# sxontheway/milliEye

Hardware: AMD Instinct MI355X
Metric: frames/sec YOLOv3-416+fusion @batch32, 1/2/4/8 MI355X; mAP@0.5 vs ref (higher is better)
Workload: dtype f32; 1 GPU; yolov3.cfg 416x416 fp32 inference, batch=32 per GPU, full milliEye: Darknet.forward -> NMS -> Network.forward mode 0 (R-CNN head + radar fusion, 2 radar boxes/frame) -> output rows, synthetic frames U[0,1), deterministic trained-like weights; stage=full, batch_per_gpu=32, global_batch=32, img_size=416, parallelism=frames sharded over 1 GPU(s), one process per GPU, no data-path collective, rccl_ranks=0, full=False, output_rows_last_step=6449, rois_last_step=6449

## Files before the change

millieye_amd/csrc/conv.hip:

```cpp
#include <stdlib.h>

#include "common.h"
#include "dma.h"

#include "conv32_common.h"

namespace me32 {
int launch_p8_tile(const ConvP& p, int tile, hipStream_t stream);
bool ws1x1_f32_eligible(const ConvP& p);
int launch_ws1x1_f32(const ConvP& p, hipStream_t stream);
bool ws3x3_f32_eligible(const ConvP& p);
int launch_ws3x3_f32(const ConvP& p, hipStream_t stream);
bool stem_mfma_eligible(const ConvP& p);
int launch_stem_mfma(const ConvP& p, hipStream_t stream);
}

namespace {

template <int BM, int BN, int BK, int WR, int WC, int ABL = 0, int PRIO = 0>
__global__ __launch_bounds__(256) void conv_igemm_f32(ConvP p) {
  static_assert(WR * WC == 4, "4 waves per workgroup");
  constexpr int TM = BM / WR, TN = BN / WC;
  constexpr int MT = TM / 32, NT = TN / 32;
  static_assert(MT >= 1 && NT >= 1, "wave tile must hold at least one 32x32 MFMA tile");
  constexpr int LP = BK + 4;
  constexpr int CH = BK / 4;
  constexpr int A_IT = (BM * CH + 255) / 256;
  constexpr int B_IT = (BN * CH + 255) / 256;

  extern __shared__ __attribute__((aligned(16))) float smem[];
  float* As = smem;
  float* Bs = smem + 2 * BM * LP;

  const int tid = threadIdx.x;
  const int lane = tid & 63;
  const int wave = tid >> 6;
  const int wr = wave / WC, wc = wave % WC;
  const int r32 = lane & 31, hh = lane >> 5;

  int tile_m, tile_n;
  {
    const int nwg = p.tiles_m * p.tiles_n;
    const int bid = blockIdx.x;
    const int q = nwg >> 3, r = nwg & 7;
    const int xcd = bid & 7, idx = bid >> 3;
    const int wg = (xcd < r ? xcd * (q + 1) : r * (q + 1) + (xcd - r) * q) + idx;
    tile_n = wg % p.tiles_n;
// ... 1305 lines not shown

extern "C" {

int64_t me_conv2d_flops(const me_conv_desc* d) {
  if (!d) return 0;
  return 2ll * d->n * d->ho * d->wo * (int64_t)d->cout * d->ksize * d->ksize * d->cin;
}

int64_t me_conv2d_workspace_bytes(const me_conv_desc* d) {
  ConvP p;
  if (!d || fill_params(d, p) != 0 || d->cin <= 4) return 0;
  if ((d->tile >= 41 && d->tile <= 45) || d->tile == 47) {
    static const int shape[7][2] = {{128, 128}, {128, 64}, {64, 64}, {128, 32}, {256, 128}, {0, 0}, {64, 64}};
    const int bm = shape[d->tile - 41][0], bn = shape[d->tile - 41][1];
    const long long tiles = (long long)((p.M + bm - 1) / bm) * ((p.cout + bn - 1) / bn);
    const int split = d->split_k > 0 ? d->split_k : 4;
    return (int64_t)(tiles % 256) * split * bm * bn * (int64_t)sizeof(float);
  }
  const ConvPlan plan = plan_conv(p, d->tile, d->split_k > 0 ? d->split_k : kMaxSplit);
  const int split = d->split_k > 0 ? d->split_k : plan.splitk;
  return split > 1 ? (int64_t)split * p.M * p.cout * (int64_t)sizeof(float) : 0;
}

int me_conv2d_f32(const me_conv_desc* d, void* stream_) {
  hipStream_t stream = reinterpret_cast<hipStream_t>(stream_);
  ConvP p;
  int rc = fill_params(d, p);
  if (rc) return rc;
  ME_REQUIRE(d->x && d->wgt && d->scale && d->shift && d->y, ME_E_NULLPTR, "me_conv2d_f32: null tensor pointer");
  ME_REQUIRE(d->upsample == 1 || d->upsample == 2, ME_E_BADARG, "me_conv2d_f32: upsample must be 1 or 2");
  ME_REQUIRE(d->act >= 0 && d->act <= 2, ME_E_BADARG, "me_conv2d_f32: unknown activation %d", d->act);
  ME_REQUIRE(d->y_pitch >= d->cout, ME_E_BADARG, "me_conv2d_f32: y_pitch < cout");

  if (d->cin <= 4) {
    ME_REQUIRE(d->ksize == 3, ME_E_BADARG, "me_conv2d_f32: cin <= 4 needs ksize 3 (direct stem kernel)");
    ME_REQUIRE(d->cout <= SC_MAXCOUT, ME_E_TOOBIG, "me_conv2d_f32: small-cin kernel supports cout <= %d", SC_MAXCOUT);
    ME_REQUIRE(d->res == nullptr && d->upsample == 1, ME_E_BADARG,
               "me_conv2d_f32: small-cin kernel has no residual/upsample epilogue");
    ME_REQUIRE(d->x_nchw || d->x_pitch >= d->cin, ME_E_BADARG, "me_conv2d_f32: x_pitch < cin");
    ME_REQUIRE(me::aligned16(d->y), ME_E_ALIGN, "me_conv2d_f32: y not 16-byte aligned");
    if (d->tile == 0 && me32::stem_mfma_eligible(p)) return me32::launch_stem_mfma(p, stream);
    if (d->cin == 3 && (d->y_pitch & 3) == 0 && d->tile != 91) {
      const unsigned mb = (unsigned)((p.M + 255) / 256);
      if (d->cout % 32 == 0) {
        hipLaunchKernelGGL(conv_stem3_f32<32>, dim3(mb, d->cout / 32), dim3(256), 0, stream, p);
        return me::check_launch("conv_stem3_f32");
      }
      if (d->cout % 16 == 0) {
        hipLaunchKernelGGL(conv_stem3_f32<16>, dim3(mb, d->cout / 16), dim3(256), 0, stream, p);
        return me::check_launch("conv_stem3_f32");
      }
    }
    const long long threads = (long long)p.M * (((p.cout + 7) & ~7) >> 3);
    const unsigned blocks = (unsigned)((threads + 255) / 256);
    if (d->cin == 3)
      hipLaunchKernelGGL(conv_smallcin_f32<3>, dim3(blocks), dim3(256), 0, stream, p);
    else
      hipLaunchKernelGGL(conv_smallcin_f32<4>, dim3(blocks), dim3(256), 0, stream, p);
    return me::check_launch("conv_smallcin_f32");
  }

  ME_REQUIRE(!d->x_nchw, ME_E_BADARG, "me_conv2d_f32: NCHW input only supported for cin <= 4");
  ME_REQUIRE(d->cin % 4 == 0, ME_E_BADARG, "me_conv2d_f32: cin %% 4 != 0 (cin=%d)", d->cin);
  ME_REQUIRE(d->x_pitch >= d->cin && d->x_pitch % 4 == 0, ME_E_ALIGN, "me_conv2d_f32: x_pitch must be >= cin, %% 4");
  ME_REQUIRE(me::aligned16(d->x) && me::aligned16(d->wgt), ME_E_ALIGN, "me_conv2d_f32: x / wgt not 16-byte aligned");
  ME_REQUIRE(!d->res || d->res_pitch >= d->cout, ME_E_BADARG, "me_conv2d_f32: res_pitch < cout");
// ... 90 lines not shown
```

millieye_amd/engine.py:

```python
import ctypes as C
import os

import torch

from . import hip

__all__ = ["DarknetEngine", "ConvWeights", "pick_tap_module", "invalidate_weights", "bump_versions"]

_ALIGN = 256

_EPOCH = [0]


def invalidate_weights():
    _EPOCH[0] += 1


def bump_versions(*tensors):
    torch.autograd.graph.increment_version(tensors)

_DTYPES = ("f32", "bf16", "f16")
_TORCH_HALF = {"bf16": torch.bfloat16, "f16": torch.float16}


def _resolve(idx, current):
    idx = int(idx)
    return current + idx if idx < 0 else idx


def pick_tap_module(module_defs):
    if len(module_defs) > 8 and module_defs[8]["type"] == "convolutional":
        return 8
    yolos = [i for i, d in enumerate(module_defs) if d["type"] == "yolo"]
    if len(yolos) < 2:
        return None
    tap = None
    for i in range(yolos[0] + 1, yolos[1]):
        d = module_defs[i]
        if d["type"] == "convolutional" and int(d["filters"]) == 256:
            tap = i
    return tap


class ConvWeights:

    def __init__(self, conv, bn=None, dtype="f32", cin_pad=0, cout_pad=0):
        self.conv, self.bn = conv, bn
        self.dtype, self.cin_pad, self.cout_pad = dtype, cin_pad, cout_pad
        self.wgt = self.scale = self.shift = None
        self.wgt_tiled = None
        self.want_rot = False
        self.rot = self.rot_tiled = None
        self.want_parity, self.parity, self.parity_stamp = False, None, None
        self._stamp = None

    def _sources(self):
        cp = self.conv._parameters
        ts = [cp["weight"]]
        if cp.get("bias") is not None:
            ts.append(cp["bias"])
        if self.bn is not None:
            bp, bb = self.bn._parameters, self.bn._buffers
            ts += [bp["weight"], bp["bias"], bb["running_mean"], bb["running_var"]]
        return ts

    def stamp(self):
        return tuple((t.data_ptr(), t._version) for t in self._sources()) + (_EPOCH[0],)

    def _prepare_packed_f32(self, device):
        conv, bn = self.conv, self.bn
        w = conv.weight
        cout, cin, k, k2 = w.shape
        if k != k2:
            return None
        srcs = [w] + [t for t in ((conv.bias,) if conv.bias is not None else ())]
        if bn is not None:
            srcs += [bn.weight, bn.bias, bn.running_mean, bn.running_var]
        if not all(t.device == device and t.dtype == torch.float32 and t.is_contiguous() for t in srcs):
            return None
        f32 = dict(device=device, dtype=torch.float32)
        realloc = self.wgt is None or self.wgt.device != device or tuple(self.wgt.shape) != (cout, k, k, cin) \
            or self.wgt.dtype != torch.float32
        if realloc:
            self.wgt = torch.empty((cout, k, k, cin), **f32)
            self.scale, self.shift = torch.empty(cout, **f32), torch.empty(cout, **f32)
            self.wgt_tiled = torch.empty((k * k, cin // 16, cout, 16), **f32) if cin % 16 == 0 else None
# ... 3 lines not shown
            self.rot_tiled = torch.empty((k * k, cout // 16, cin, 16), **f32) if cout % 16 == 0 else None
        if realloc:
            self.parity = None
        if self.want_parity and k == 3 and self.parity is None:
            self.parity = torch.empty((4 * cin, 2, 2, cout), **f32)
        return "realloc" if realloc else True

    def _pack_desc(self, d):
        conv, bn = self.conv, self.bn
        ptr = lambda t: t.data_ptr() if t is not None else None
        cout, cin, k, _ = conv.weight.shape
        d.w, d.bias = conv.weight.data_ptr(), ptr(conv.bias)
        d.gamma, d.beta = ptr(bn.weight if bn is not None else None), ptr(bn.bias if bn is not None else None)
        d.mean, d.var = ptr(bn.running_mean if bn is not None else None), ptr(bn.running_var if bn is not None else None)
        d.ohwi, d.tiled = self.wgt.data_ptr(), ptr(self.wgt_tiled)
        d.rot, d.rot_tiled = ptr(self.rot if self.want_rot else None), ptr(self.rot_tiled if self.want_rot else None)
        d.scale, d.shift = self.scale.data_ptr(), self.shift.data_ptr()
        d.parity = ptr(self.parity if self.want_parity else None)
        d.cout, d.cin, d.ksize, d.eps = cout, cin, k, float(bn.eps) if bn is not None else 0.0
        return d

    def _refresh_packed_f32(self, device):
        done = self._prepare_packed_f32(device)
        if done is None:
            return None
        self.parity_stamp = None
        d = self._pack_desc(hip.PackDesc())
        hip.check(hip.lib().me_pack_conv_f32(d.w, d.cout, d.cin, d.ksize, d.bias, d.gamma, d.beta, d.mean, d.var, d.eps, d.ohwi,
                                             d.tiled, d.rot, d.rot_tiled, d.scale, d.shift, hip.stream_ptr()),
                  "me_pack_conv_f32")
        return done

    def refresh(self, device):
        stamp = self.stamp() + (self.want_rot,)
        if stamp == self._stamp and self.wgt is not None and self.wgt.device == device:
            return False
        dev = torch.device(device)
        if self.dtype == "f32" and not self.cin_pad and not self.cout_pad and dev.type == "cuda":
            if dev.index is None:
                dev = torch.device("cuda", torch.cuda.current_device())
            done = self._refresh_packed_f32(dev)
            if done is not None:
                self._stamp = stamp
                return done
        with torch.no_grad():
            w = self.conv.weight.detach().to(device=device, dtype=torch.float32)
            packed = w.permute(0, 2, 3, 1).contiguous()
            cout = w.shape[0]
            if self.bn is not None:
                g = self.bn.weight.detach().to(device, torch.float64)
                b = self.bn.bias.detach().to(device, torch.float64)
                mean = self.bn.running_mean.detach().to(device, torch.float64)
                var = self.bn.running_var.detach().to(device, torch.float64)
                scale = g / torch.sqrt(var + self.bn.eps)
                shift = b - mean * scale
                if self.conv.bias is not None:
                    shift = shift + self.conv.bias.detach().to(device, torch.float64) * scale
            else:
                scale = torch.ones(cout, dtype=torch.float64, device=device)
                if self.conv.bias is not None:
                    shift = self.conv.bias.detach().to(device, torch.float64)
                else:
                    shift = torch.zeros(cout, dtype=torch.float64, device=device)
            scale, shift = scale.to(torch.float32), shift.to(torch.float32)
            cin = packed.shape[3]
            if self.cin_pad > cin:
# ... 401 lines not shown
        plan.arena = torch.empty(max(total, _ALIGN), dtype=torch.uint8, device=device)
        if plan.arena.data_ptr() % _ALIGN:
            raise RuntimeError("the caching allocator returned an arena that is not 256-byte aligned")
        plan.arena_bytes = total
        plan.dtype = self.dtype
        plan.rows = sum(yolo_rows)
        plan.num_classes = None
        base = plan.arena.data_ptr()

        def view(tt):
            root, coff = tt.root()
            return base + root.offset + tt.esize * coff, root.c

        def typed_view(tt, nchw):
            root, coff = tt.root()
            flat = plan.arena.view(_TORCH_HALF[self.dtype] if tt.esize == 2 else torch.float32)
            pitch, off = root.c, root.offset // tt.esize + coff
            if nchw:
                return torch.as_strided(flat, (n, tt.c, tt.h, tt.w), (tt.h * tt.w * pitch, 1, tt.w * pitch, pitch), off)
            return torch.as_strided(flat, (n, tt.h, tt.w, tt.c), (tt.h * tt.w * pitch, tt.w * pitch, pitch, 1), off)

        lib = hip.lib()
        launches = []
        plan.input_descs = []
        plan.yolo_raw = []
        plan.yolo_descs = []
        plan.conv_descs = []
        flops = 0
        for op in ops:
            kind = op["kind"]
            if kind == "conv":
                x, y = op["x"], op["y"]
                cw = self._conv_weights(op["module"], x.c if x.padded else 0, y.c if y.padded else 0)
                if cw.refresh(device) == "realloc" and self._plans:
                    self._plans.clear()
                dsc = hip.Conv16Desc() if bf16 else hip.ConvDesc()
                if x.external:
                    dsc.x, dsc.x_pitch, dsc.x_nchw = None, x.c, 1
                    plan.input_descs.append(dsc)
                else:
                    dsc.x, dsc.x_pitch = view(x)
                    dsc.x_nchw = 0
                dsc.wgt, dsc.scale, dsc.shift = cw.wgt.data_ptr(), cw.scale.data_ptr(), cw.shift.data_ptr()
                if op["res"] is not None:
                    dsc.res, dsc.res_pitch = view(op["res"])
                else:
                    dsc.res, dsc.res_pitch = None, 0
                dsc.y, dsc.y_pitch = view(y)
                dsc.n, dsc.h, dsc.w, dsc.cin = n, x.h, x.w, x.c
                dsc.cout, dsc.ksize, dsc.stride, dsc.pad = cw.wgt.shape[0], op["k"], op["s"], op["pad"]
                dsc.ho, dsc.wo, dsc.act, dsc.upsample, dsc.tile = op["ho"], op["wo"], op["act"], op["ups"], 0
                dsc.split_k, dsc.workspace, dsc.workspace_bytes = 0, None, 0
                dsc.wgt_tiled = cw.wgt_tiled.data_ptr() if cw.wgt_tiled is not None else None
                if bf16:
                    dsc.y_f32 = 1 if y.esize == 4 else 0
                    dsc.half_type = half_type
                op["launch"] = len(launches)
                op["desc"] = dsc
                launches.append((lib.me_conv2d_h16 if bf16 else lib.me_conv2d_f32, (C.byref(dsc),), dsc,
                                 f"conv{op['module']}"))
                plan.conv_descs.append((op["module"], dsc))
                flops += 2 * n * op["ho"] * op["wo"] * op["cout"] * op["k"] * op["k"] * (x.c - x.padded)
            elif kind == "pool" and bf16:
                x, y = op["x"], op["y"]
                (xp, xpitch), (yp, ypitch) = view(x), view(y)
                launches.append((lib.me_maxpool_h16,
                                 (xp, xpitch, yp, ypitch, n, x.h, x.w, x.c, op["k"], op["s"],
                                  0 if op["zero_ext"] else op["pad"], op["zero_ext"], op["ho"], op["wo"], half_type), None,
                                 f"pool{op['module']}"))
            elif kind == "pool":
                x, y = op["x"], op["y"]
                dsc = hip.PoolDesc()
                dsc.x, dsc.x_pitch = view(x)
                dsc.y, dsc.y_pitch = view(y)
                dsc.n, dsc.h, dsc.w, dsc.c = n, x.h, x.w, x.c
                dsc.size, dsc.stride, dsc.pad, dsc.zero_ext = op["k"], op["s"], (0 if op["zero_ext"] else op["pad"]), \
                    op["zero_ext"]
                dsc.ho, dsc.wo = op["ho"], op["wo"]
                launches.append((lib.me_maxpool_f32, (C.byref(dsc),), dsc, f"pool{op['module']}"))
            elif kind == "upsample":
                x, y = op["x"], op["y"]
                (xp, xpitch), (yp, ypitch) = view(x), view(y)
                launches.append((lib.me_upsample_h16 if x.esize == 2 else lib.me_upsample_f32,
                                 (xp, xpitch, yp, ypitch, n, x.h, x.w, x.c, op["f"]), None,
                                 f"upsample{op['module']}"))
            elif kind == "add":
# ... 190 lines not shown
    def __enter__(self):
        _GRAPH_SCOPE.depth = getattr(_GRAPH_SCOPE, "depth", 0) + 1
        return self

    def __exit__(self, *exc):
        _GRAPH_SCOPE.depth = getattr(_GRAPH_SCOPE, "depth", 1) - 1
        return False


def _graphs_enabled():
    import os
    return getattr(_GRAPH_SCOPE, "depth", 0) > 0 or os.environ.get("MILLIEYE_HIPGRAPH", "0") in ("1", "true", "on")


_TUNE_CACHE = {}
_TUNE_FILE_LOADED = [False]
_TUNE_STATS = {"measured": 0, "synced": 0}
_TUNE_TILES = (1, 2, 3, 4, 5)
_TUNE_SPLITS = (1, 2, 3, 4, 6, 8)
_KW_MAX_POSITIONS = 6144
_TUNE_TILES_BF16 = (1, 2, 3, 4, 11, 12, 13, 14, 15)
_TILE_SHAPES_BF16 = {40: (32, 32), 41: (32, 64),
                     1: (128, 128), 2: (128, 64), 3: (64, 64), 4: (256, 128),
                     11: (128, 128), 12: (128, 64), 13: (64, 64), 14: (256, 128), 15: (192, 128),
                     100: (128, 256), 110: (192, 256), 120: (256, 256), 101: (128, 128), 121: (256, 128), 131: (384, 128),
                     141: (512, 128), 200: (128, 256), 201: (128, 128), 221: (256, 128), 301: (128, 128), 311: (192, 128),
                     321: (256, 128), 331: (256, 128), 421: (256, 128), 431: (384, 128), 441: (512, 128),
                     621: (256, 128), 721: (256, 128), 731: (384, 128),
                     810: (192, 256), 820: (256, 256), 821: (256, 128), 831: (384, 128), 841: (512, 128),
                     1210: (192, 256), 1221: (256, 128), 1231: (384, 128),
                     50: (32, 256),
                     60: (256, 128)}
_TUNE_TILES_TAIL = (41, 42, 43, 44, 45)
_TUNE_TILES_P8_F32 = (201, 221)
_TUNE_TILES_P8 = (100, 110, 120, 101, 121, 131, 141, 200, 201, 221, 311, 321, 421, 431, 441,
                  621, 721, 731, 810, 831, 1210, 1231)


_SPECULATIVE = os.environ.get("MILLIEYE_CHECK_FIRST", "0") != "1"


def _autotune_enabled():
    import os
    return os.environ.get("MILLIEYE_AUTOTUNE", "1") not in ("0", "false", "off")


def _tune_file():
    import os
    path = os.environ.get("MILLIEYE_TUNE_CACHE")
    if path:
        return path
    base = os.environ.get("XDG_CACHE_HOME", os.path.join(os.path.expanduser("~"), ".cache"))
    return os.path.join(base, "millieye_amd", "conv_tune_v15.json")


def _tune_load():
    import json
    import os
    if _TUNE_FILE_LOADED[0]:
        return
    _TUNE_FILE_LOADED[0] = True
    try:
        with open(_tune_file()) as fh:
            for k, v in json.load(fh).items():
                _TUNE_CACHE[tuple(int(x) for x in k.split(","))] = (int(v[0]), int(v[1]))
    except (OSError, ValueError):
        pass


def _tune_save():
    import json
    import os
    path = _tune_file()
    try:
        os.makedirs(os.path.dirname(path), exist_ok=True)
        tmp = f"{path}.{os.getpid()}.tmp"
        with open(tmp, "w") as fh:
            json.dump({",".join(str(int(x)) for x in k): list(v) for k, v in _TUNE_CACHE.items()}, fh)
        os.replace(tmp, path)
    except OSError:
        pass


def _autotune(plan, lib):
    import os
    import time

    stream = hip.stream_ptr()
    _tune_load()
    bf16 = plan.dtype in _TORCH_HALF
    conv_fn = lib.me_conv2d_h16 if bf16 else lib.me_conv2d_f32
    todo, keyed = [], []
    for _m, d in plan.conv_descs:
        if d.cin <= 4:
            continue
        key = (d.n, d.h, d.w, d.cin, d.cout, d.ksize, d.stride, d.upsample, int(bool(d.res)))
        if bf16:
            key += (16 + d.y_f32 + 2 * d.half_type,)
        keyed.append((key, d))
        hit = _TUNE_CACHE.get(key)
        if hit is not None:
            d.tile, d.split_k = hit
        else:
            todo.append((key, d))

    def agree_on_rank0():
        import torch.distributed as dist
        if not (dist.is_available() and dist.is_initialized() and dist.get_world_size() > 1):
            return
        if os.environ.get("MILLIEYE_TUNE_SYNC", "0") not in ("1", "true", "on"):
            return
        box = [{k: (int(dd.tile), int(dd.split_k)) for k, dd in keyed} if dist.get_rank() == 0 else None]
        dist.broadcast_object_list(box, src=0)
        _TUNE_STATS["synced"] += 1
        for k, dd in keyed:
            hit0 = box[0].get(k)
            if hit0 is not None:
                dd.tile, dd.split_k = hit0
                _TUNE_CACHE[k] = hit0

    def ensure_workspace(nbytes):
        have = plan.conv_ws.numel() - 256 if plan.conv_ws is not None else 0
        if nbytes > have:
            plan.conv_ws = torch.empty(nbytes + 256, dtype=torch.uint8, device=plan.arena.device)
            have = nbytes
        ptr = plan.conv_ws.data_ptr() + (-plan.conv_ws.data_ptr()) % 256 if plan.conv_ws is not None else None
        for _m2, d2 in plan.conv_descs:
            if d2.cin > 4:
                d2.workspace, d2.workspace_bytes = ptr, have
        return have

    def scratch_of(d2):
        if not bf16 and d2.tile in _TUNE_TILES_TAIL + (47,):
            return int(lib.me_conv2d_workspace_bytes(C.byref(d2)))
        if bf16 and d2.tile >= 100:
            return int(lib.me_conv2d_h16_workspace_bytes(C.byref(d2)))
        return d2.split_k * d2.n * d2.ho * d2.wo * d2.cout * 4 if d2.split_k > 1 else 0

    def required():
        return max([scratch_of(d2) for _m2, d2 in plan.conv_descs if d2.cin > 4] + [0])

    _TUNE_STATS["measured"] += len(todo)
    if not todo:
        agree_on_rank0()
        ensure_workspace(required())
        return
    ws_bytes = plan.conv_ws.numel() - 256 if plan.conv_ws is not None else 0
    need = 0
    for _k, d in todo:
        slab = d.n * d.ho * d.wo * d.cout * 4
        if slab * 2 <= 512 * 2 ** 20:
            need = max(need, min(8 * slab, 512 * 2 ** 20))
        need = max(need, (128 if bf16 else 64) * 2 ** 20)
    ws_bytes = ensure_workspace(max(need, required()))

    def run(d, reps):
        for _ in range(reps):
            rc = conv_fn(C.byref(d), stream)
            if rc != 0:
                return False
        return True

    def timed(d, reps):
        a, b = torch.cuda.Event(enable_timing=True), torch.cuda.Event(enable_timing=True)
        a.record()
        ok = run(d, reps)
        b.record()
        torch.cuda.synchronize()
        return a.elapsed_time(b) / reps if ok else None

    t_end = time.perf_counter() + 0.3
    d0 = todo[0][1]
    d0.tile, d0.split_k = 0, 1
    while time.perf_counter() < t_end:
        run(d0, 5)
        torch.cuda.synchronize()
    for key, d in todo:
        hit = _TUNE_CACHE.get(key)
        if hit is not None:
            d.tile, d.split_k = hit
            continue
        slab = d.n * d.ho * d.wo * d.cout * 4
        stages = d.ksize * d.ksize * ((d.cin + 15) // 16)
        best = (float("inf"), 0, 1)
        cands = []
        tiles = _TUNE_TILES
        if bf16:
            stages = d.ksize * d.ksize * (d.cin // 32)
            tiles = _TUNE_TILES_BF16 if d.cin % 64 == 0 else _TUNE_TILES_BF16[:4] + (15,)
            if d.ksize == 3 and d.stride == 1 and d.upsample == 1 and d.wgt_tiled and not d.y_f32:
                tiles = tiles + _TUNE_TILES_P8
            no_ws = os.environ.get("MILLIEYE_NO_WS", "")
            if d.ksize == 1 and d.stride == 1 and d.upsample == 1 and not d.y_f32 and not d.res and "50" not in no_ws:
                tiles = tiles + (50,)
            if d.ksize == 3 and d.cin <= 64 and d.upsample == 1 and not d.y_f32 and "60" not in no_ws:
                tiles = tiles + (60,)
            if d.n * d.ho * d.wo <= _KW_MAX_POSITIONS and os.environ.get("MILLIEYE_NO_KW", "0") != "1":
                tiles = tiles + (40, 41)
        else:
            if d.cin % 16 == 0 and os.environ.get("MILLIEYE_TUNE_TAIL", "1") != "0":
                tiles = tiles + _TUNE_TILES_TAIL
            if d.ksize == 3 and d.stride == 1 and d.upsample == 1 and d.wgt_tiled:
                tiles = tiles + _TUNE_TILES_P8_F32
            no_ws32 = os.environ.get("MILLIEYE_NO_WS32", "")
            if d.ksize == 1 and d.stride == 1 and d.upsample == 1 and not d.res and d.act != hip.ACT_SIGMOID \
                    and d.cin in (64, 128, 256, 384, 512) and "50" not in no_ws32:
                tiles = tiles + (50,)
            if d.ksize == 3 and d.pad == 1 and d.cin in (32, 64) and d.upsample == 1 and d.act != hip.ACT_SIGMOID \
                    and "60" not in no_ws32:
                tiles = tiles + (60,)
        for tile in tiles:
            bm, bn = _TILE_SHAPES_BF16[tile] if (bf16 or tile >= 100 or tile in (50, 60)) else \
                {1: (128, 128), 2: (128, 64), 3: (64, 64), 4: (128, 32), 5: (256, 128), 7: (64, 64)}[tile % 40]
            ntiles = -(-d.n * d.ho * d.wo // bm) * -(-d.cout // bn)
            tail = not bf16 and tile in _TUNE_TILES_TAIL
            if tail and ntiles % 256 == 0:
                continue
            p8_split = False
            for split in (_TUNE_SPLITS[1:] if tail else (1,) if tile in (50, 60) or (bf16 and tile in (40, 41)) else _TUNE_SPLITS if tile < 100
                          else (1, 2, 3, 4) if p8_split else (1,)):
                d.tile, d.split_k = tile, split
                if tail or (tile >= 100 and split > 1):
                    if split > stages or scratch_of(d) > ws_bytes:
                        continue
                elif split > 1 and (split * slab > ws_bytes or ntiles * split > 4096 or split > stages):
                    continue
                if not run(d, 2):
                    continue
                ms = timed(d, 4)
                if ms is not None:
                    cands.append((ms, tile, split, split > 1 or tail))
        cands.sort()
        finalists = cands[:4]
        whole = [c for c in cands if not c[3]]
        if whole and whole[0] not in finalists:
            finalists.append(whole[0])
        score = {}
        for _round in range(3):
            for c in finalists:
                d.tile, d.split_k = c[1], c[2]
                ms = timed(d, 6)
                if ms is not None:
                    score.setdefault(c, []).append(ms)
        ranked = sorted((sorted(v)[len(v) // 2], c) for c, v in score.items())
        if os.environ.get("MILLIEYE_TUNE_VERBOSE"):
            import sys
            print("[tune]", key, " ".join(f"{c[1]}/{c[2]}:{1e3 * c[0]:.0f}>{1e3 * t:.0f}us" for t, c in ranked), file=sys.stderr, flush=True)
        if ranked:
            best = ranked[0]
            whole = [r for r in ranked if not r[1][3]]
            if best[1][3] and whole and best[0] > 0.98 * whole[0][0]:
                best = whole[0]
            best = (best[0], best[1][1], best[1][2])
        d.tile, d.split_k = best[1], best[2]
        _TUNE_CACHE[key] = (best[1], best[2])
    agree_on_rank0()
    ensure_workspace(required())
    _tune_save()


def _bneck_mode():
    return os.environ.get("MILLIEYE_BNECK", "1")


_BNECK_CACHE = {}
_BNECK_STATS = {"fused": 0, "kept": 0}


def _fuse_bottlenecks(plan, ops, lib):
    import time
    stream = hip.stream_ptr()
    launches = plan.launches
    conv_ops = [op for op in ops if op["kind"] == "conv"]
    index = {id(op): k for k, op in enumerate(ops)}
    pairs = []
    for a, b in zip(conv_ops, conv_ops[1:]):
        da, db = a["desc"], b["desc"]
        if not (index[id(b)] == index[id(a)] + 1 and b["x"] is a["y"]):
            continue
        mid = a["y"]
        if mid.readers != [index[id(b)]] or mid.pinned or mid.parent is not None or mid.padded or mid.esize != 2:
            continue
        if not (da.ksize == 1 and da.stride == 1 and da.upsample == 1 and not da.res and not da.y_f32 and not da.x_nchw
                and db.ksize == 3 and db.stride == 1 and db.pad == 1 and db.upsample == 1 and not db.y_f32
                and da.wgt_tiled and db.wgt_tiled and da.cout == db.cin and da.y_pitch == db.x_pitch):
            continue
        bd = hip.Bneck16Desc()
# ... 78 lines not shown
```

millieye_amd/hip.py:

```python
import ctypes as C
import os

import torch

__all__ = ["lib", "available", "default_device", "MeError"]

_HERE = os.path.dirname(os.path.abspath(__file__))
LIB_PATH = os.environ.get("MILLIEYE_HIP_LIB") or os.path.join(_HERE, "libmillieye_hip.so")

ACT_LINEAR, ACT_LEAKY, ACT_SIGMOID = 0, 1, 2


class MeError(RuntimeError):
    pass


class ConvDesc(C.Structure):
    _fields_ = [
        ("x", C.c_void_p), ("wgt", C.c_void_p), ("scale", C.c_void_p), ("shift", C.c_void_p),
        ("res", C.c_void_p), ("y", C.c_void_p),
        ("x_pitch", C.c_int64), ("res_pitch", C.c_int64), ("y_pitch", C.c_int64),
        ("n", C.c_int32), ("h", C.c_int32), ("w", C.c_int32), ("cin", C.c_int32),
        ("cout", C.c_int32), ("ksize", C.c_int32), ("stride", C.c_int32), ("pad", C.c_int32),
        ("ho", C.c_int32), ("wo", C.c_int32),
# ... 372 lines not shown
        raise MeError(f"{name} must be NHWC-contiguous or a channel slice of an NHWC-contiguous tensor")
    return pitch


def conv2d(x_nhwc, wgt_packed, scale, shift, ksize, stride, pad, act, residual=None, upsample=1, out=None,
           x_nchw=False, tile=0, split_k=0, wgt_tiled=None, in_launch_reduce=False, tap_masks=None):
    _require_cuda_f32(x_nhwc, "x")
    if x_nchw:
        n, cin, h, w = x_nhwc.shape
    else:
        n, h, w, cin = x_nhwc.shape
    cout = wgt_packed.shape[0]
    ho = (h + 2 * pad - ksize) // stride + 1
    wo = (w + 2 * pad - ksize) // stride + 1
    if out is None:
        out = torch.empty((n, ho * upsample, wo * upsample, cout), device=x_nhwc.device, dtype=torch.float32)
    d = ConvDesc()
    d.x, d.wgt, d.scale, d.shift = x_nhwc.data_ptr(), wgt_packed.data_ptr(), scale.data_ptr(), shift.data_ptr()
    d.res = residual.data_ptr() if residual is not None else None
    d.y = out.data_ptr()
    d.x_pitch = cin
    if not x_nchw and not x_nhwc.is_contiguous():
        pitch = x_nhwc.stride(2)
        if x_nhwc.stride() != (h * w * pitch, w * pitch, pitch, 1):
            raise MeError("x must be NHWC-contiguous or a channel slice of an NHWC-contiguous tensor")
        d.x_pitch = pitch
    d.res_pitch = _nhwc_pitch(residual, "residual") if residual is not None else 0
    d.y_pitch = _nhwc_pitch(out, "out")
    d.n, d.h, d.w, d.cin, d.cout = n, h, w, cin, cout
    d.ksize, d.stride, d.pad, d.ho, d.wo = ksize, stride, pad, ho, wo
    d.act, d.upsample, d.x_nchw, d.tile, d.split_k = act, upsample, 1 if x_nchw else 0, tile, split_k
    if tile >= 100 and wgt_tiled is None and wgt_packed.shape[3] % 16 == 0:
        wgt_tiled = tile_weights_f32(wgt_packed)
    d.wgt_tiled = wgt_tiled.data_ptr() if wgt_tiled is not None else None
    if tap_masks is not None:
        d.tap_mask_cols = int(tap_masks[0])
        for i, m in enumerate(tap_masks[1]):
            d.tap_mask[i] = int(m)
        d.split_k = 1
    need = lib().me_conv2d_workspace_bytes(C.byref(d)) if tap_masks is None else 0
    keep = None
    if need > 0:
        ws_ptr, keep = _workspace(need, x_nhwc.device, slot="conv")
        d.workspace, d.workspace_bytes = ws_ptr, need
        if in_launch_reduce:
            d.tile_counters, d.tile_counters_len, _keep2 = tile_counters(x_nhwc.device)
    check(lib().me_conv2d_f32(C.byref(d), stream_ptr()), "me_conv2d_f32")
    return out


_CONV_AUTO = {}
_CONV_AUTO_LOADED = [False]


def _conv_auto_file():
    base = os.environ.get("MILLIEYE_TUNE_CACHE")
    if base:
        return base + ".train"
    root = os.environ.get("XDG_CACHE_HOME", os.path.join(os.path.expanduser("~"), ".cache"))
    try:
        gpu = torch.cuda.get_device_name(torch.cuda.current_device()).replace(" ", "_").replace("/", "_")
    except Exception:
        gpu = "unknown"
    return os.path.join(root, "millieye_amd", f"conv_auto_v2_abi{int(lib().me_abi_version())}_{gpu}.json")


# ... 48 lines not shown
                for _ in range(2):
                    scratch = conv2d(x_nhwc, wgt_packed, scale, shift, ksize, stride, pad, act, residual=residual, out=scratch,
                                     tile=tile, split_k=split, wgt_tiled=wgt_tiled, tap_masks=tm)
                a, b = torch.cuda.Event(enable_timing=True), torch.cuda.Event(enable_timing=True)
                a.record()
                for _ in range(3):
                    conv2d(x_nhwc, wgt_packed, scale, shift, ksize, stride, pad, act, residual=residual, out=scratch, tile=tile,
                           split_k=split, wgt_tiled=wgt_tiled, tap_masks=tm)
                b.record()
                torch.cuda.synchronize()
                ms = a.elapsed_time(b) / 3
            except MeError:
                continue
            if ms < best[0]:
                best = (ms, tile, split, masked)
        hit = _CONV_AUTO[key] = (best[1], best[2], best[3])
        _conv_auto_save()
    masked = len(hit) > 2 and hit[2]
    try:
        return conv2d(x_nhwc, wgt_packed, scale, shift, ksize, stride, pad, act, residual=residual, out=out, tile=hit[0],
                      split_k=hit[1], wgt_tiled=wgt_tiled, tap_masks=tap_masks if masked else None)
    except MeError:
        if hit[0] == 0 and not masked:
            raise
        _CONV_AUTO[key] = (0, 0, 0)
        return conv2d(x_nhwc, wgt_packed, scale, shift, ksize, stride, pad, act, residual=residual, out=out, wgt_tiled=wgt_tiled)


def tile_weights_f32(wgt_packed):
    cout, kh, kw, cin = wgt_packed.shape
    if cin % 16:
        raise MeError("tile_weights_f32: cin must be a multiple of 16")
    return wgt_packed.reshape(cout, kh * kw, cin // 16, 16).permute(1, 2, 0, 3).contiguous()


def tile_weights_h16(wgt_packed):
    cout, kh, kw, cin = wgt_packed.shape
    if cin % 32:
        raise MeError("tile_weights_h16: cin must be a multiple of 32")
    return wgt_packed.reshape(cout, kh * kw, cin // 32, 32).permute(1, 2, 0, 3).contiguous()


def conv2d_h16(x, wgt_packed, scale, shift, ksize, stride, pad, act, residual=None, upsample=1, out=None,
                x_nchw=False, y_f32=False, tile=0, split_k=0, half=torch.bfloat16, wgt_tiled=None, debug_ws=None, tap_masks=None):
    if not (isinstance(x, torch.Tensor) and x.is_cuda):
        raise MeError("x must be a CUDA tensor")
    if x_nchw:
        n, cin, h, w = x.shape
    else:
        n, h, w, cin = x.shape
    if cin > 4:
        half = x.dtype
    if half not in HALF_TYPES:
        raise MeError(f"me_conv2d_h16: 16-bit type must be bfloat16 or float16 (got {half})")
    want = torch.float32 if cin <= 4 else half
    if x.dtype != want or wgt_packed.dtype != want:
        raise MeError(f"me_conv2d_h16: x / wgt must be {want} for cin={cin} (got {x.dtype} / {wgt_packed.dtype})")
    cout = wgt_packed.shape[0]
    ho = (h + 2 * pad - ksize) // stride + 1
    wo = (w + 2 * pad - ksize) // stride + 1
    odt = torch.float32 if y_f32 else half
    if out is None:
        out = torch.empty((n, ho * upsample, wo * upsample, cout), device=x.device, dtype=odt)
    if out.dtype != odt or (residual is not None and residual.dtype != odt):
        raise MeError("me_conv2d_h16: out / residual dtype does not match y_f32")
    d = Conv16Desc()
# ... 403 lines not shown
```

Before: 1879 frames/s.

## Add Winograd F(2,3) fp32 MFMA conv kernel as autotune candidate for 3x3 layers

Adds a Winograd F(2,3) kernel for 3x3 stride-1 convolutions, applied in one dimension along width. It pairs adjacent output columns, transforms the input on the fly from LDS, and runs four MFMA products per pair against pre-transformed weights. The transformed weights are built in float64 on the host side and cached per layer. The engine then offers tiles 70-72 to the autotuner, which is on by default through MILLIEYE_WINO. The aim is to cut multiplies along the width axis by 4/6, at the cost of extra weight memory, more complex pipelining and some change in fp32 rounding.

```diff
diff --git a/millieye_amd/csrc/conv.hip b/millieye_amd/csrc/conv.hip
--- a/millieye_amd/csrc/conv.hip
+++ b/millieye_amd/csrc/conv.hip
@@ -13,6 +13,7 @@
 int launch_ws3x3_f32(const ConvP& p, hipStream_t stream);
 bool stem_mfma_eligible(const ConvP& p);
 int launch_stem_mfma(const ConvP& p, hipStream_t stream);
+int launch_wino_f32(const ConvP& p, int tile, int split_k, hipStream_t stream);
 }
 
 namespace {
@@ -1384,6 +1385,8 @@
   ME_REQUIRE(d->act >= 0 && d->act <= 2, ME_E_BADARG, "me_conv2d_f32: unknown activation %d", d->act);
   ME_REQUIRE(d->y_pitch >= d->cout, ME_E_BADARG, "me_conv2d_f32: y_pitch < cout");
 
+  if (d->tile >= 70 && d->tile <= 72) return me32::launch_wino_f32(p, d->tile, d->split_k, stream);
+
   if (d->cin <= 4) {
     ME_REQUIRE(d->ksize == 3, ME_E_BADARG, "me_conv2d_f32: cin <= 4 needs ksize 3 (direct stem kernel)");
     ME_REQUIRE(d->cout <= SC_MAXCOUT, ME_E_TOOBIG, "me_conv2d_f32: small-cin kernel supports cout <= %d", SC_MAXCOUT);
diff --git a/millieye_amd/csrc/conv_wino_f32.hip b/millieye_amd/csrc/conv_wino_f32.hip
--- /dev/null
+++ b/millieye_amd/csrc/conv_wino_f32.hip
@@ -0,0 +1,297 @@
+#include "conv32_common.h"
+
+namespace {
+using namespace me_dma;
+
+__device__ __forceinline__ unsigned udiv_magic32(unsigned n, unsigned m, unsigned s) { return (__umulhi(n, m) + n) >> s; }
+
+template <int N, class F, int I = 0>
+__device__ __forceinline__ void static_for(F&& f) {
+  if constexpr (I < N) {
+    f(std::integral_constant<int, I>{});
+    static_for<N, F, I + 1>(static_cast<F&&>(f));
+  }
+}
+
+template <int BP, int BN, int WR, int WC>
+__global__ __launch_bounds__(64 * WR * WC, 1) void conv_wino_f32(ConvP p) {
+  constexpr int NW = WR * WC;
+  static_assert(BP == 32 * WR && BN == 32 * WC, "one 32 pairs x 32 couts x 4 positions block per wave");
+  constexpr int BK = 16, NST = 3;
+  constexpr int GA = 4 * BP / 16, GB = 4 * BN / 16;
+  static_assert(GA % NW == 0 && GB % NW == 0, "groups must split evenly over the waves");
+  constexpr int LA = GA / NW, LB = GB / NW, LPW = LA + LB;
+  static_assert(LA % 4 == 0 && LB >= 1 && LB <= 4, "the A loads go out in blocks of four, the B loads in one block");
+  constexpr int STAGE_F = (GA + GB) * 256;
+  constexpr unsigned STAGE_B = STAGE_F * 4u;
+
+  extern __shared__ __attribute__((aligned(16))) float smem[];
+  const unsigned lds_base = (unsigned)(unsigned long long)(__attribute__((address_space(3))) float*)smem;
+
+  const int tid = threadIdx.x;
+  const int lane = tid & 63;
+  const int wave = __builtin_amdgcn_readfirstlane(tid >> 6);
+  const int wr = wave / WC, wc = wave % WC;
+  const int r32 = lane & 31, hh = lane >> 5;
+  const int J = p.sps, hj = p.ho * J;
+
+  int tile_m, tile_n;
+  {
+    const int nwg = p.tiles_m * p.tiles_n;
+    const int bid = blockIdx.x;
+    const int q = nwg >> 3, r = nwg & 7;
+    const int xcd = bid & 7, idx = bid >> 3;
+    const int t = (xcd < r ? xcd * (q + 1) : r * (q + 1) + (xcd - r) * q) + idx;
+    const int per_panel = p.tiles_m * p.gn;
+    const int panel = t / per_panel;
+    const int rr = t - panel * per_panel;
+    const int left = p.tiles_n - panel * p.gn;
+    const int width = left < p.gn ? left : p.gn;
+    tile_m = rr / width;
+    tile_n = panel * p.gn + (rr - tile_m * width);
+    tile_m = __builtin_amdgcn_readfirstlane(tile_m);
+    tile_n = __builtin_amdgcn_readfirstlane(tile_n);
+  }
+  const int m0 = tile_m * BP, n0 = tile_n * BN;
+
+  const int img0 = (int)udiv_magic32((unsigned)m0, p.hw_m, p.hw_s);
+  const long long img_elems = (long long)p.h * p.w * p.x_pitch;
+  const long long bias_elems = ((long long)p.w + 1) * p.x_pitch;
+  const u32x4 rsrc_a = make_rsrc(p.x + (long long)img0 * img_elems - bias_elems);
+  const u32x4 rsrc_b = make_rsrc(p.wgt_tiled + (long long)n0 * 16);
+  const unsigned b_step = (unsigned)p.cout * 64u;
+
+  const int lrow = lane >> 2;
+  unsigned v_a[3][LA];
+  unsigned v_b[LB];
+#pragma unroll
+  for (int j = 0; j < LA; ++j) {
+    const int row = (wave + NW * j) * 16 + lrow;
+    const int d = row / BP, pl = row % BP;
+    const int q = (lane & 3) ^ ((row >> 2) & 3);
+    unsigned base = kOobOffset, ok = 0;
+    const int m = m0 + pl;
+    if (m < p.M) {
+      const int nimg = (int)udiv_magic32((unsigned)m, p.hw_m, p.hw_s);
+      const int rem = m - nimg * hj;
+      const int oy = (int)udiv_magic32((unsigned)rem, p.wo_m, p.wo_s), jj = rem - oy * J;
+      const int col = 2 * jj - 1 + d;
+      if ((unsigned)col < (unsigned)p.w) {
+        const long long e = (long long)(nimg - img0) * img_elems + ((long long)(oy - 1) * p.w + col) * p.x_pitch + bias_elems;
+        base = (unsigned)(e * 4) + 16u * q;
+        ok = ((unsigned)(oy - 1) < (unsigned)p.h ? 1u : 0u) | 2u | ((unsigned)(oy + 1) < (unsigned)p.h ? 4u : 0u);
+      }
+    }
+#pragma unroll
+    for (int ky = 0; ky < 3; ++ky) v_a[ky][j] = ((ok >> ky) & 1u) ? base : kOobOffset;
+  }
+#pragma unroll
+  for (int j = 0; j < LB; ++j) {
+    const int row = (wave + NW * j) * 16 + lrow;
+    const int pp = row / BN, cl = row % BN;
+    const int q = (lane & 3) ^ ((row >> 2) & 3);
+    v_b[j] = n0 + cl < p.cout ? ((unsigned)pp * (unsigned)p.cs * (unsigned)p.cout + (unsigned)cl) * 64u + 16u * q : kOobOffset;
+  }
+
+  f32x16 acc[4];
+#pragma unroll
+  for (int i = 0; i < 4; ++i)
+#pragma unroll
+    for (int e = 0; e < 16; ++e) acc[i][e] = 0.f;
+
+  const unsigned wave_lds = __builtin_amdgcn_readfirstlane(lds_base + (unsigned)wave * 1024u);
+  const unsigned pitch4 = (unsigned)p.x_pitch * 4u;
+  const int sw = (r32 >> 2) & 3;
+  const int off0 = ((0 + hh) ^ sw) * 4, off1 = ((2 + hh) ^ sw) * 4;
+  const float* a_frag = smem + (wr * 32 + r32) * BK;
+  const float* b_frag = smem + (4 * BP + wc * 32 + r32) * BK;
+
+  unsigned a_ky[3], b_ky[3];
+#pragma unroll
+  for (int ky = 0; ky < 3; ++ky) {
+    a_ky[ky] = (unsigned)(ky * p.w) * pitch4;
+    b_ky[ky] = (unsigned)(ky * 4) * (unsigned)p.cs * b_step;
+  }
+
+  auto issue = [&](auto ky_c, unsigned ca, unsigned cb, unsigned dst) {
+    constexpr int KY = decltype(ky_c)::value;
+    const unsigned sa = __builtin_amdgcn_readfirstlane(a_ky[KY] + ca), sb = __builtin_amdgcn_readfirstlane(b_ky[KY] + cb);
+    static_for<LA / 4>([&](auto o_c) {
+      constexpr int O = decltype(o_c)::value * 4;
+      dma_same<4, NW * 1024, O>(v_a[KY], rsrc_a, sa, dst + (unsigned)O * (NW * 1024u));
+    });
+    dma_same<LB, NW * 1024, 0>(v_b, rsrc_b, sb, dst + (unsigned)LA * (NW * 1024u));
+  };
+
+  struct Frag {
+    float4 d[2][4], u[2][4];
+  };
+  auto read_frags = [&](int slot, Frag& f) {
+    const float* Ab = a_frag + slot * STAGE_F;
+    const float* Bb = b_frag + slot * STAGE_F;
+#pragma unroll
+    for (int half = 0; half < 2; ++half) {
+      const int off = half ? off1 : off0;
+#pragma unroll
+      for (int i = 0; i < 4; ++i) f.d[half][i] = *reinterpret_cast<const float4*>(Ab + i * BP * BK + off);
+#pragma unroll
+      for (int i = 0; i < 4; ++i) f.u[half][i] = *reinterpret_cast<const float4*>(Bb + i * BN * BK + off);
+    }
+  };
+  auto multiply_half = [&](const float4 (&v)[4], const float4 (&u)[4]) {
+#pragma unroll
+    for (int kk = 0; kk < 4; ++kk)
+#pragma unroll
+      for (int i = 0; i < 4; ++i) {
+        const float4 av = v[i], bv = u[i];
+        const float a = kk == 0 ? av.x : kk == 1 ? av.y : kk == 2 ? av.z : av.w;
+        const float b = kk == 0 ? bv.x : kk == 1 ? bv.y : kk == 2 ? bv.z : bv.w;
+        acc[i] = __builtin_amdgcn_mfma_f32_32x32x2f32(a, b, acc[i], 0, 0, 0);
+      }
+  };
+
+  unsigned ca = 0, cb = 0;
+  auto step = [&](auto ky_c, auto last_c, const Frag& cur, Frag& nxt) {
+    constexpr int KY = decltype(ky_c)::value;
+    constexpr bool LAST = decltype(last_c)::value;
+    float4 v[2][4];
+#pragma unroll
+    for (int half = 0; half < 2; ++half) {
+      const float4 d0 = cur.d[half][0], d1 = cur.d[half][1], d2 = cur.d[half][2], d3 = cur.d[half][3];
+      v[half][0] = make_float4(d0.x - d2.x, d0.y - d2.y, d0.z - d2.z, d0.w - d2.w);
+      v[half][1] = make_float4(d1.x + d2.x, d1.y + d2.y, d1.z + d2.z, d1.w + d2.w);
+      v[half][2] = make_float4(d2.x - d1.x, d2.y - d1.y, d2.z - d1.z, d2.w - d1.w);
+      v[half][3] = make_float4(d1.x - d3.x, d1.y - d3.y, d1.z - d3.z, d1.w - d3.w);
+    }
+    multiply_half(v[0], cur.u[0]);
+    __builtin_amdgcn_sched_barrier(0);
+    if constexpr (!(LAST && KY == 2)) {
+      constexpr int YOUNGER = (LAST && KY == 1) ? 0 : 1;
+      asm volatile("s_waitcnt vmcnt(%0) lgkmcnt(0)" ::"n"(LPW * YOUNGER) : "memory");
+      __builtin_amdgcn_s_barrier();
+      asm volatile("" ::: "memory");
+      if constexpr (!LAST) issue(ky_c, ca + BK * 4u, cb + b_step, wave_lds + KY * STAGE_B);
+      read_frags((KY + 1) % 3, nxt);
+    }
+    __builtin_amdgcn_sched_barrier(0);
+    multiply_half(v[1], cur.u[1]);
+    __builtin_amdgcn_sched_barrier(0);
+  };
+  static_assert(NST == 3, "the slot of a stage is its filter row");
+  static_for<3>([&](auto ky_c) { issue(ky_c, ca, cb, wave_lds + decltype(ky_c)::value * STAGE_B); });
+  Frag f0, f1;
+  asm volatile("s_waitcnt vmcnt(%0)" ::"n"(LPW * 2) : "memory");
+  __builtin_amdgcn_s_barrier();
+  asm volatile("" ::: "memory");
+  read_frags(0, f0);
+  for (int c = 0; c + 1 < p.cs; ++c) {
+    step(std::integral_constant<int, 0>{}, std::false_type{}, f0, f1);
+    step(std::integral_constant<int, 1>{}, std::false_type{}, f1, f0);
+    step(std::integral_constant<int, 2>{}, std::false_type{}, f0, f1);
+    f0 = f1;
+    ca += BK * 4u;
+    cb += b_step;
+  }
+  step(std::integral_constant<int, 0>{}, std::true_type{}, f0, f1);
+  step(std::integral_constant<int, 1>{}, std::true_type{}, f1, f0);
+  step(std::integral_constant<int, 2>{}, std::true_type{}, f0, f1);
+
+  const int co = n0 + wc * 32 + r32;
+  if (co >= p.cout) return;
+  const float sc = p.scale[co], sh = p.shift[co];
+#pragma unroll
+  for (int e = 0; e < 16; ++e) {
+    const int m = m0 + wr * 32 + (e & 3) + 8 * (e >> 2) + 4 * hh;
+    if (m >= p.M) continue;
+    const int nimg = (int)udiv_magic32((unsigned)m, p.hw_m, p.hw_s);
+    const int rem = m - nimg * hj;
+    const int oy = (int)udiv_magic32((unsigned)rem, p.wo_m, p.wo_s), ox = 2 * (rem - oy * J);
+    const long long pix = ((long long)nimg * p.ho + oy) * p.wo + ox;
+    const float m1 = acc[1][e], m2 = acc[2][e];
+    float y0 = apply_act((acc[0][e] + m1 + m2) * sc + sh, p.act);
+    float y1 = apply_act((m1 - m2 - acc[3][e]) * sc + sh, p.act);
+    const bool second = ox + 1 < p.wo;
+    if (p.res) {
+      const float* rp = p.res + pix * p.res_pitch + co;
+      y0 += rp[0];
+      if (second) y1 += rp[p.res_pitch];
+    }
+    float* yp = p.y + pix * p.y_pitch + co;
+    me::store4(yp, y0, p.store_mode);
+    if (second) me::store4(yp + p.y_pitch, y1, p.store_mode);
+  }
+}
+
+void magic_u32(unsigned d, unsigned* m, unsigned* s) {
+  unsigned sh = 0;
+  while ((1ull << sh) < d) ++sh;
+  *s = sh;
+  *m = (unsigned)(((1ull << 32) * ((1ull << sh) - d)) / d + 1);
+}
+
+template <int BP>
+bool wino_addressable(const ConvP& p) {
+  const long long J = (p.wo + 1) / 2;
+  const long long span_imgs = (BP - 1) / ((long long)p.ho * J) + 2;
+  const long long img_bytes = (long long)p.h * p.w * p.x_pitch * 4;
+  const long long row_bytes = (3ll * p.w + 4) * p.x_pitch * 4 + (long long)p.cin * 4;
+  const long long a_max = span_imgs * img_bytes + 2 * row_bytes;
+  const long long b_max = 12ll * p.cin * p.cout * 4 + 256ll * 64;
+  return a_max < (1ll << 31) && b_max < (1ll << 31);
+}
+
+template <int BP, int BN, int WR, int WC>
+int launch_wino(ConvP p, hipStream_t stream) {
+  ME_REQUIRE(wino_addressable<BP>(p), ME_E_TOOBIG, "me_conv2d_f32: tile %d needs every input / weight offset below 2^31",
+             BP == 128 ? 72 : BN == 64 ? 70 : 71);
+  const int J = (p.wo + 1) / 2;
+  const long long pairs = (long long)p.n * p.ho * J;
+  p.M = (int)pairs;
+  p.sps = J;
+  magic_u32((unsigned)(p.ho * J), &p.hw_m, &p.hw_s);
+  magic_u32((unsigned)J, &p.wo_m, &p.wo_s);
+  p.cs = p.cin / 16;
+  p.stages = 3 * p.cs;
+  p.tiles_m = (int)((pairs + BP - 1) / BP);
+  p.tiles_n = (p.cout + BN - 1) / BN;
+  const long long col_bytes = (long long)BN * 12 * p.cin * 4;
+  const long long panel_bytes = 1300ll * 1024;
+  p.gn = p.tiles_n;
+  if (col_bytes * p.tiles_n > panel_bytes) {
+    const long long fit = panel_bytes / col_bytes;
+    p.gn = fit < 1 ? 1 : fit > p.tiles_n ? p.tiles_n : (int)fit;
+  }
+  constexpr int NW = WR * WC;
+  const size_t lds = (size_t)3 * (4 * BP + 4 * BN) * 64;
+  auto kern = conv_wino_f32<BP, BN, WR, WC>;
+  static bool attr_set = false;
+  if (!attr_set) {
+    ME_HIP(hipFuncSetAttribute(reinterpret_cast<const void*>(kern), hipFuncAttributeMaxDynamicSharedMemorySize, (int)lds));
+    attr_set = true;
+  }
+  const long long blocks = (long long)p.tiles_m * p.tiles_n;
+  ME_REQUIRE(blocks < (1ll << 31), ME_E_TOOBIG, "me_conv2d_f32: grid too large");
+  hipLaunchKernelGGL(kern, dim3((unsigned)blocks), dim3(64 * NW), lds, stream, p);
+  return me::check_launch("conv_wino_f32");
+}
+
+}
+
+namespace me32 {
+
+int launch_wino_f32(const ConvP& p, int tile, int split_k, hipStream_t stream) {
+  ME_REQUIRE(p.ks == 3 && p.stride == 1 && p.pad == 1 && p.ups == 1 && !p.x_nchw && p.cin % 16 == 0 && split_k <= 1 &&
+                 p.mask_cols == 0,
+             ME_E_BADARG,
+             "me_conv2d_f32: tile %d (Winograd F(2,3)) needs a 3x3 / stride 1 / pad 1 layer, NHWC input, cin %% 16 == 0, no "
+             "upsample, no split-K, no tap masks", tile);
+  ME_REQUIRE(p.wgt_tiled != nullptr, ME_E_NULLPTR, "me_conv2d_f32: tile %d reads its Winograd weight packing from wgt_tiled", tile);
+  ME_REQUIRE(me::aligned16(p.wgt_tiled) && me::aligned16(p.x) && p.x_pitch % 4 == 0 && p.x_pitch >= p.cin, ME_E_ALIGN,
+             "me_conv2d_f32: tile %d needs 16-byte aligned x / wgt_tiled and x_pitch %% 4 == 0, >= cin", tile);
+  ME_REQUIRE(!p.res || p.res_pitch >= p.cout, ME_E_BADARG, "me_conv2d_f32: res_pitch < cout");
+  if (tile == 70) return launch_wino<64, 64, 2, 2>(p, stream);
+  if (tile == 72) return launch_wino<128, 64, 4, 2>(p, stream);
+  return launch_wino<64, 32, 2, 1>(p, stream);
+}
+
+}
diff --git a/millieye_amd/engine.py b/millieye_amd/engine.py
--- a/millieye_amd/engine.py
+++ b/millieye_amd/engine.py
@@ -52,6 +52,7 @@
         self.want_rot = False
         self.rot = self.rot_tiled = None
         self.want_parity, self.parity, self.parity_stamp = False, None, None
+        self.want_wino, self.wgt_wino, self._wino_stamp = False, None, None
         self._stamp = None
 
     def _sources(self):
@@ -121,6 +122,20 @@
         return done
 
     def refresh(self, device):
+        done = self._refresh(device)
+        if self.want_wino and self.wgt is not None and self.wgt.dtype == torch.float32:
+            stamp = self.stamp()
+            if stamp != self._wino_stamp or self.wgt_wino is None or self.wgt_wino.device != self.wgt.device:
+                with torch.no_grad():
+                    wino = hip.wino_weights_f32(self.wgt)
+                if self.wgt_wino is None or self.wgt_wino.shape != wino.shape or self.wgt_wino.device != wino.device:
+                    self.wgt_wino = wino
+                else:
+                    self.wgt_wino.copy_(wino)
+                self._wino_stamp = stamp
+        return done
+
+    def _refresh(self, device):
         stamp = self.stamp() + (self.want_rot,)
         if stamp == self._stamp and self.wgt is not None and self.wgt.device == device:
             return False
@@ -588,6 +603,10 @@
             if kind == "conv":
                 x, y = op["x"], op["y"]
                 cw = self._conv_weights(op["module"], x.c if x.padded else 0, y.c if y.padded else 0)
+                wino = (not bf16 and _wino_mode() != "0" and op["k"] == 3 and op["s"] == 1 and op["pad"] == 1 and op["ups"] == 1
+                        and not x.external and x.c % 16 == 0 and not x.padded and not y.padded)
+                if wino and not cw.want_wino:
+                    cw.want_wino, cw._wino_stamp = True, None
                 if cw.refresh(device) == "realloc" and self._plans:
                     self._plans.clear()
                 dsc = hip.Conv16Desc() if bf16 else hip.ConvDesc()
@@ -608,6 +627,8 @@
                 dsc.ho, dsc.wo, dsc.act, dsc.upsample, dsc.tile = op["ho"], op["wo"], op["act"], op["ups"], 0
                 dsc.split_k, dsc.workspace, dsc.workspace_bytes = 0, None, 0
                 dsc.wgt_tiled = cw.wgt_tiled.data_ptr() if cw.wgt_tiled is not None else None
+                if wino and cw.wgt_wino is not None:
+                    dsc._packings = (dsc.wgt_tiled, cw.wgt_wino.data_ptr())
                 if bf16:
                     dsc.y_f32 = 1 if y.esize == 4 else 0
                     dsc.half_type = half_type
@@ -864,12 +885,23 @@
                      50: (32, 256),
                      60: (256, 128)}
 _TUNE_TILES_TAIL = (41, 42, 43, 44, 45)
-_TUNE_TILES_P8_F32 = (201, 221)
+_TUNE_TILES_WINO = (70, 71, 72)
+_TUNE_TILES_P8_F32 = (201, 221) + _TUNE_TILES_WINO
 _TUNE_TILES_P8 = (100, 110, 120, 101, 121, 131, 141, 200, 201, 221, 311, 321, 421, 431, 441,
                   621, 721, 731, 810, 831, 1210, 1231)
 
 
 _SPECULATIVE = os.environ.get("MILLIEYE_CHECK_FIRST", "0") != "1"
+
+
+def _wino_mode():
+    return os.environ.get("MILLIEYE_WINO", "1")
+
+
+def _point_weights(d):
+    packs = getattr(d, "_packings", None)
+    if packs is not None:
+        d.wgt_tiled = packs[1] if d.tile in _TUNE_TILES_WINO else packs[0]
 
 
 def _autotune_enabled():
@@ -929,10 +961,16 @@
         key = (d.n, d.h, d.w, d.cin, d.cout, d.ksize, d.stride, d.upsample, int(bool(d.res)))
         if bf16:
             key += (16 + d.y_f32 + 2 * d.half_type,)
+        can_wino = getattr(d, "_packings", None) is not None
+        if can_wino and _wino_mode() == "force":
+            key += (70,)
         keyed.append((key, d))
         hit = _TUNE_CACHE.get(key)
+        if hit is not None and hit[0] in _TUNE_TILES_WINO and not can_wino:
+            hit = None
         if hit is not None:
             d.tile, d.split_k = hit
+            _point_weights(d)
         else:
             todo.append((key, d))
 
@@ -949,6 +987,7 @@
             hit0 = box[0].get(k)
             if hit0 is not None:
                 dd.tile, dd.split_k = hit0
+                _point_weights(dd)
                 _TUNE_CACHE[k] = hit0
 
     def ensure_workspace(nbytes):
@@ -1004,13 +1043,16 @@
     t_end = time.perf_counter() + 0.3
     d0 = todo[0][1]
     d0.tile, d0.split_k = 0, 1
+    _point_weights(d0)
     while time.perf_counter() < t_end:
         run(d0, 5)
         torch.cuda.synchronize()
     for key, d in todo:
         hit = _TUNE_CACHE.get(key)
-        if hit is not None:
+        can_wino = getattr(d, "_packings", None) is not None
+        if hit is not None and (can_wino or hit[0] not in _TUNE_TILES_WINO):
             d.tile, d.split_k = hit
+            _point_weights(d)
             continue
         slab = d.n * d.ho * d.wo * d.cout * 4
         stages = d.ksize * d.ksize * ((d.cin + 15) // 16)
@@ -1033,7 +1075,7 @@
             if d.cin % 16 == 0 and os.environ.get("MILLIEYE_TUNE_TAIL", "1") != "0":
                 tiles = tiles + _TUNE_TILES_TAIL
             if d.ksize == 3 and d.stride == 1 and d.upsample == 1 and d.wgt_tiled:
-                tiles = tiles + _TUNE_TILES_P8_F32
+                tiles = tiles + tuple(t for t in _TUNE_TILES_P8_F32 if t not in _TUNE_TILES_WINO)
             no_ws32 = os.environ.get("MILLIEYE_NO_WS32", "")
             if d.ksize == 1 and d.stride == 1 and d.upsample == 1 and not d.res and d.act != hip.ACT_SIGMOID \
                     and d.cin in (64, 128, 256, 384, 512) and "50" not in no_ws32:
@@ -1041,17 +1083,21 @@
             if d.ksize == 3 and d.pad == 1 and d.cin in (32, 64) and d.upsample == 1 and d.act != hip.ACT_SIGMOID \
                     and "60" not in no_ws32:
                 tiles = tiles + (60,)
+            if can_wino:
+                tiles = _TUNE_TILES_WINO if _wino_mode() == "force" else tiles + _TUNE_TILES_WINO
         for tile in tiles:
-            bm, bn = _TILE_SHAPES_BF16[tile] if (bf16 or tile >= 100 or tile in (50, 60)) else \
+            bm, bn = _TILE_SHAPES_BF16[tile] if (bf16 or tile >= 100 or tile in (50, 60)) else (64, 64) if tile in _TUNE_TILES_WINO else \
                 {1: (128, 128), 2: (128, 64), 3: (64, 64), 4: (128, 32), 5: (256, 128), 7: (64, 64)}[tile % 40]
             ntiles = -(-d.n * d.ho * d.wo // bm) * -(-d.cout // bn)
             tail = not bf16 and tile in _TUNE_TILES_TAIL
             if tail and ntiles % 256 == 0:
                 continue
             p8_split = False
-            for split in (_TUNE_SPLITS[1:] if tail else (1,) if tile in (50, 60) or (bf16 and tile in (40, 41)) else _TUNE_SPLITS if tile < 100
+            for split in (_TUNE_SPLITS[1:] if tail else (1,) if tile in (50, 60) or (bf16 and tile in (40, 41))
+                          or (not bf16 and tile in _TUNE_TILES_WINO) else _TUNE_SPLITS if tile < 100
                           else (1, 2, 3, 4) if p8_split else (1,)):
                 d.tile, d.split_k = tile, split
+                _point_weights(d)
                 if tail or (tile >= 100 and split > 1):
                     if split > stages or scratch_of(d) > ws_bytes:
                         continue
@@ -1071,6 +1117,7 @@
         for _round in range(3):
             for c in finalists:
                 d.tile, d.split_k = c[1], c[2]
+                _point_weights(d)
                 ms = timed(d, 6)
                 if ms is not None:
                     score.setdefault(c, []).append(ms)
@@ -1085,6 +1132,7 @@
                 best = whole[0]
             best = (best[0], best[1][1], best[1][2])
         d.tile, d.split_k = best[1], best[2]
+        _point_weights(d)
         _TUNE_CACHE[key] = (best[1], best[2])
     agree_on_rank0()
     ensure_workspace(required())
diff --git a/millieye_amd/hip.py b/millieye_amd/hip.py
--- a/millieye_amd/hip.py
+++ b/millieye_amd/hip.py
@@ -428,6 +428,8 @@
     d.act, d.upsample, d.x_nchw, d.tile, d.split_k = act, upsample, 1 if x_nchw else 0, tile, split_k
     if tile >= 100 and wgt_tiled is None and wgt_packed.shape[3] % 16 == 0:
         wgt_tiled = tile_weights_f32(wgt_packed)
+    if tile in (70, 71, 72) and wgt_tiled is None and ksize == 3 and wgt_packed.shape[3] % 16 == 0:
+        wgt_tiled = wino_weights_f32(wgt_packed)
     d.wgt_tiled = wgt_tiled.data_ptr() if wgt_tiled is not None else None
     if tap_masks is not None:
         d.tap_mask_cols = int(tap_masks[0])
@@ -542,6 +544,16 @@
     if cin % 16:
         raise MeError("tile_weights_f32: cin must be a multiple of 16")
     return wgt_packed.reshape(cout, kh * kw, cin // 16, 16).permute(1, 2, 0, 3).contiguous()
+
+
+def wino_weights_f32(wgt_packed):
+    cout, kh, kw, cin = wgt_packed.shape
+    if (kh, kw) != (3, 3) or cin % 16:
+        raise MeError("wino_weights_f32: 3x3 filters with cin a multiple of 16")
+    g = wgt_packed.to(torch.float64)
+    g0, g1, g2 = g[:, :, 0], g[:, :, 1], g[:, :, 2]
+    u = torch.stack((g0, (g0 + g1 + g2) / 2, (g0 - g1 + g2) / 2, g2), dim=2)
+    return u.reshape(cout, 3, 4, cin // 16, 16).permute(1, 2, 3, 0, 4).to(torch.float32).contiguous()
 
 
 def tile_weights_h16(wgt_packed):
```

After: 1878 frames/s. No clear change (-0.1%).
